# HuiHuiLan/Clustering-Hidden-Markov-Models-with-Variational-Bayesian-Hierarchical-EM

Measured on AMD Instinct MI355X. Metric: VBHEM E-steps/sec (whole node), N baseHMMs × K clusters × S states; ELBO match, higher is better.
Workload: dtype f64; 1 GPU; C4: N=100000 base HMMs, K=16 clusters, S=8 states, Sb=8, d=8, full cov, tau=10, Nv=100; N=100000, K=16, S=8, Sb=8, d=8, tau=10, parallelism=bases sharded over 1 GPU(s), 1 RCCL all-reduce/E-step

## Files before the change

### clustering-hidden-markov-models-with-variational-bayesian-hierarchical-em_amd/csrc/vbhem_em.hip

```cpp
#include <hip/hip_runtime.h>

#include <cfloat>
#include <chrono>
#include <cmath>
#include <cstdlib>
#include <map>
#include <mutex>
#include <string>
#include <vector>

#include "vbhem_em.h"
#include "vbhem_em_deriv_terms.h"
#include "vbhem_em_dev.h"
#include "vbhem_em_host.h"
#include "vbhem_em_trial_ctrl.h"
#include "vbhem_internal.h"
#include "vbhem_special.h"

namespace {

constexpr double kPi = 3.14159265358979323846;

using vbhem::psi_recur;

// ... 596 lines not shown
    if (std::isnan(L)) {
      L = -INFINITY;
      *stable = 0;
      break;
    }
    bool do_break = false;
    if (it > 1 && std::fabs((L - lastL) / lastL) <= opt->minDiff) do_break = true;
    if (it == opt->max_iter) do_break = true;
    LogLs[it] = L;
    ++it;
    lastL = L;
    if (do_break) break;
  }
  *iters = it;
  *L_final = L;
  if (deriv) {
    if (*stable) return derivs_at(&pre.t, opt, ext->dLL);
    nan_derivs(opt, d, ext->dLL);
  }
  return VBHEM_OK;
}

using MappedBuf = vbhem::EmMappedBuf;
std::map<int, std::vector<MappedBuf>> g_mapped_bufs;

hipError_t acquire_mapped_buf(size_t bytes, MappedBuf &m) {
  int dev = 0;
  hipError_t e = hipGetDevice(&dev);
  if (e != hipSuccess) return e;
  {
    std::lock_guard<std::mutex> g(g_mapped_mu);
    auto &v = g_mapped_bufs[dev];
    for (size_t x = 0; x < v.size(); ++x)
      if (v[x].bytes >= bytes) {
        m = v[x];
        v.erase(v.begin() + (long)x);
        return hipSuccess;
      }
    if (!v.empty()) {
      (void)hipHostFree(v.back().h);
      v.pop_back();
    }
  }
  m.bytes = (bytes + 4095) / 4096 * 4096;
  e = hipHostMalloc(reinterpret_cast<void **>(&m.h), m.bytes, hipHostMallocMapped);
  if (e == hipSuccess) e = hipHostGetDevicePointer(reinterpret_cast<void **>(&m.d), m.h, 0);
  return e;
}

void release_mapped_buf(const MappedBuf &m) {
  if (!m.h) return;
  int dev = 0;
  if (hipGetDevice(&dev) != hipSuccess) return;
  std::lock_guard<std::mutex> g(g_mapped_mu);
  g_mapped_bufs[dev].push_back(m);
}

size_t post_len(int K, int S, int d, size_t dd) {
  return (size_t)K + 3 * (size_t)K * S + (size_t)K * S * S + (size_t)K * S * d + (size_t)K * S * dd;
}

size_t trials_ws_doubles(int N, int K, int S, int d, size_t dd, int R, size_t slen, int nW) {
  const size_t KS = (size_t)K * S, nd = (size_t)VBHEM_DLL_LEN(d, nW);
  const size_t consts = KS * S + KS + KS * d + KS * dd + KS + (size_t)K;
  return (size_t)R * (2 * consts + 2 * post_len(K, S, d, dd) + 2 * KS + KS * 13 + 2 * slen +
                      2 * (size_t)N * K + (size_t)vbhem::hyp_table_len(d) + nd * KS + nd) +
         ((size_t)R * sizeof(vbhem::TrialCtrl) + 7) / 8 + ((size_t)R * sizeof(int) + 7) / 8;
}

const char *trials_unsupported(const vbhem_base_t *base, int K, int S, int R) {
  if (R < 1 || K < 1 || S < 1) return "R, KT and S must be positive";
  if ((long long)R * K > 256) return "R * KT > 256 (vbhem_estep_fused_trials)";
  if (S > 16) return "S > 16 (vbhem_estep_fused_trials)";
  if (base->SB > S) return "Sb > S (vbhem_estep_fused_trials)";
  if (!vbhem::em_dev_supported(base->d, S)) return "d > 16 (the device-side EM math)";
  return nullptr;
}

}

extern "C++" {
namespace vbhem {
hipError_t em_wait_flag(const int *flag, int seq, hipStream_t st) { return wait_flag(flag, seq, st); }
hipError_t em_acquire_mapped_buf(size_t bytes, EmMappedBuf &m) { return acquire_mapped_buf(bytes, m); }
void em_release_mapped_buf(const EmMappedBuf &m) { release_mapped_buf(m); }
}
}

int vbhem_em_run_ext(const vbhem_base_t *base, const double *tildeN_dev, int T,
                     const vbhem_em_opt_t *opt, vbhem_post_t *post, double *LogLs, int *iters,
                     double *L_final, int *stable, double *stats_dev, double *hatZ_dev,
                     double *LL_dev, void *workspace_dev, size_t workspace_bytes, void *stream,
                     vbhem_allreduce_fn allreduce, void *allreduce_ctx, const vbhem_em_ext_t *ext) {
  if (!base || !post_ok(post) || !opt_ok(opt, post->d) || !LogLs || !iters || !L_final ||
      !stable || !stats_dev || post->d != base->d || post->covmode != base->covmode)
    return VBHEM_ERR_ARG;
  if (ext && ext->rccl_comm && allreduce)
    return vbhem::set_error(VBHEM_ERR_ARG, "vbhem_em_run_ext: an RCCL communicator and an all-reduce callback");
  const int K = post->K, S = post->S, d = post->d;
  const size_t dd = post->covmode == VBHEM_COV_FULL ? (size_t)d * d : (size_t)d;
  const size_t need = vbhem_em_workspace_bytes(base, K, S, T);
  if (need == 0 || !workspace_dev || workspace_bytes < need) return VBHEM_ERR_WORKSPACE;
  hipStream_t st = static_cast<hipStream_t>(stream);
  if (!vbhem::em_dev_supported(d, S) || vbhem::switches().EM_HOST_MATH)
    return em_run_host(base, tildeN_dev, T, opt, post, LogLs, iters, L_final, stable, stats_dev,
                       hatZ_dev, LL_dev, workspace_dev, st, allreduce, allreduce_ctx, ext);
  vbhem_cluster_t c0 = {K, S, nullptr, nullptr, nullptr, nullptr, nullptr};
  const size_t fused = (vbhem_fused_workspace_bytes(base, &c0, T) + 255) / 256 * 256;
  const size_t nA = (size_t)K * S * S, nPi = (size_t)K * S, nm = (size_t)K * S * d,
               nP = (size_t)K * S * dd, nc = (size_t)K * S;
  double *dc = reinterpret_cast<double *>(static_cast<char *>(workspace_dev) + fused);
  vbhem_cluster_t cl = {K, S, dc, dc + nA, dc + nA + nPi, dc + nA + nPi + nm,
                        dc + nA + nPi + nm + nP};
  double *dlogOmega = dc + nA + nPi + nm + nP + nc;
  double *p = dlogOmega + K;
  PostDev pd[3];
  for (int x = 0; x < 3; ++x) pd[x] = carve_post(p, K, S, d, dd);
  double *dlLT = p; p += nc;
  double *dlogdetW = p; p += nc;
  double *dm0 = p; p += d;
  double *dW0inv = p; p += (size_t)d * d;
  double *dpart = p; p += (size_t)K * S * 13;
  int *dticket = reinterpret_cast<int *>(p); p += 1;
  double *hz[2] = {hatZ_dev, p}, *ll[2] = {LL_dev, p + (size_t)base->N * K};
  std::vector<double> W0inv;
  w0_inv(opt, d, W0inv);
  vbhem::EmDevArgs a{};
  a.K = K; a.S = S; a.d = d; a.covmode = post->covmode; a.NU = (int)vbhem_stats_nu(d, post->covmode);
  a.stats = stats_dev;
  a.alpha0 = opt->alpha0; a.eta0 = opt->eta0; a.epsilon0 = opt->epsilon0; a.lambda0 = opt->lambda0;
  a.v0 = opt->v0;
  bound_constants(opt, K, S, d, W0inv, a.logCalpha0, a.logCeta0, a.logCepsilon0, a.logB0);
  a.m0 = dm0; a.W0inv = dW0inv;
  a.logA = dc; a.logPi = dc + nA; a.cm = dc + nA + nPi; a.P = dc + nA + nPi + nm;
  a.c = dc + nA + nPi + nm + nP; a.lLT = dlLT; a.logOmega = dlogOmega; a.logdetW = dlogdetW;
  a.part = dpart; a.ticket = dticket;
  hipError_t e = hipMemcpyAsync(dm0, opt->m0, d * sizeof(double), hipMemcpyHostToDevice, st);
  if (e == hipSuccess)
    e = hipMemcpyAsync(dW0inv, W0inv.data(), W0inv.size() * sizeof(double), hipMemcpyHostToDevice, st);
  if (e == hipSuccess) e = copy_post(post, pd[0], dd, hipMemcpyHostToDevice, st);
  if (e == hipSuccess) e = hipMemsetAsync(dticket, 0, sizeof(int), st);
  Mapped mb;
  if (e == hipSuccess) e = acquire_mapped(mb);
  double *Lh = mb.h, *Ld = mb.d;
  int *flag_h = Lh ? reinterpret_cast<int *>(Lh + 2) : nullptr;
  if (flag_h) flag_h[0] = flag_h[1] = 0;
  auto set_post = [&a](const PostDev &in, const PostDev &out) {
    a.alpha = in.alpha; a.eta = in.eta; a.eps = in.eps; a.lam = in.lam; a.v = in.v; a.m = in.m;
    a.W = in.W;
    a.alpha_o = out.alpha; a.eta_o = out.eta; a.eps_o = out.eps; a.lam_o = out.lam; a.v_o = out.v;
    a.m_o = out.m; a.W_o = out.W;
  };
  set_post(pd[0], pd[1]);
  if (e == hipSuccess) e = vbhem::launch_em_dev(a, vbhem::kEmPrelude, nullptr, st);
  const size_t slen = vbhem_stats_len(K, S, d, post->covmode);
  int rc = VBHEM_OK;
  auto enqueue = [&](int j) -> bool {
    rc = vbhem_estep_fused(base, &cl, T, tildeN_dev, dlogOmega, stats_dev, hz[j % 2], ll[j % 2],
                           workspace_dev, fused, st);
    if (rc != VBHEM_OK) return false;
    rc = reduce_stats(ext, allreduce, allreduce_ctx, stats_dev, slen, st);
    if (rc != VBHEM_OK) return false;
    set_post(pd[j % 3], pd[(j + 1) % 3]);
    a.seq = j + 1;
    a.flag = reinterpret_cast<int *>(Ld + 2) + (j % 2);
    void *t0 = vbhem::timing_begin(st);
    e = vbhem::launch_em_dev(a, vbhem::kEmIterate, Ld + (j % 2), st);
    vbhem::timing_end_em_math(t0, st);
    return e == hipSuccess;
  };
  double lastL = -DBL_MAX, L = -INFINITY;
  int it = 0, fin_post = 0, fin_e = 0;
  *stable = 1;
  bool ok = e == hipSuccess && enqueue(0);
  while (ok) {
    if (it + 1 <= opt->max_iter && !enqueue(it + 1)) break;
    e = wait_flag(flag_h + (it % 2), it + 1, st);
    if (e != hipSuccess) break;
    if (ext && ext->iter_seconds) ext->iter_seconds[it] = now_s();
    L = Lh[it % 2];
    fin_e = it % 2;
    if (std::isnan(L)) {
      L = -INFINITY;
      *stable = 0;
      fin_post = it % 3;
      break;
    }
    bool do_break = false;
    if (it > 1 && std::fabs((L - lastL) / lastL) <= opt->minDiff) do_break = true;
    if (it == opt->max_iter) do_break = true;
    LogLs[it] = L;
    ++it;
    lastL = L;
    fin_post = it % 3;
    if (do_break) break;
  }
  hipError_t e2 = hipStreamSynchronize(st);
  if (e == hipSuccess) e = e2;
  if (e == hipSuccess && rc == VBHEM_OK && fin_e == 1 && base->N > 0) {
    e = hipMemcpyAsync(hatZ_dev, hz[1], (size_t)base->N * K * sizeof(double),
                       hipMemcpyDeviceToDevice, st);
    if (e == hipSuccess)
      e = hipMemcpyAsync(LL_dev, ll[1], (size_t)base->N * K * sizeof(double),
                         hipMemcpyDeviceToDevice, st);
  }
  const bool deriv = ext && ext->calc_deriv && ext->dLL;
  HostPost pre;
  if (deriv && *stable && it >= 1) pre.size_like(post);
  if (e == hipSuccess && rc == VBHEM_OK) e = copy_post(post, pd[fin_post], dd, hipMemcpyDeviceToHost, st);
  if (e == hipSuccess && rc == VBHEM_OK && deriv && *stable && it >= 1)
    e = copy_post(&pre.t, pd[(it - 1) % 3], dd, hipMemcpyDeviceToHost, st);
  if (e == hipSuccess && rc == VBHEM_OK) e = hipStreamSynchronize(st);
  if (e == hipSuccess) release_mapped(mb);
  if (rc != VBHEM_OK) return rc;
  if (e != hipSuccess) return VBHEM_ERR_HIP;
  *iters = it;
  *L_final = L;
  if (deriv) {
    if (*stable && it >= 1) return derivs_at(&pre.t, opt, ext->dLL);
    nan_derivs(opt, d, ext->dLL);
  }
  return VBHEM_OK;
}

int vbhem_em_run(const vbhem_base_t *base, const double *tildeN_dev, int T,
                 const vbhem_em_opt_t *opt, vbhem_post_t *post, double *LogLs, int *iters,
                 double *L_final, int *stable, double *stats_dev, double *hatZ_dev,
                 double *LL_dev, void *workspace_dev, size_t workspace_bytes, void *stream,
                 vbhem_allreduce_fn allreduce, void *allreduce_ctx) {
  return vbhem_em_run_ext(base, tildeN_dev, T, opt, post, LogLs, iters, L_final, stable, stats_dev,
                          hatZ_dev, LL_dev, workspace_dev, workspace_bytes, stream, allreduce,
                          allreduce_ctx, nullptr);
}

size_t vbhem_em_trials_hyp_workspace_bytes(const vbhem_base_t *base, int KT, int S, int R, int T,
                                           int W0_len) {
  if (!base || trials_unsupported(base, KT, S, R)) return 0;
  const int d = base->d;
  if (W0_len != 1 && W0_len != d) return 0;
  const size_t dd = base->covmode == VBHEM_COV_FULL ? (size_t)d * d : (size_t)d;
  vbhem_cluster_t c = {R * KT, S, nullptr, nullptr, nullptr, nullptr, nullptr};
  const size_t fused = vbhem_fused_trials_workspace_bytes(base, &c, R, T);
  if (fused == 0) return 0;
  const size_t slen = vbhem_stats_len(KT, S, d, base->covmode);
  return (fused + 255) / 256 * 256 +
         trials_ws_doubles(base->N, KT, S, d, dd, R, slen, W0_len) * sizeof(double) + 256;
}

size_t vbhem_em_trials_workspace_bytes(const vbhem_base_t *base, int KT, int S, int R, int T) {
  return base ? vbhem_em_trials_hyp_workspace_bytes(base, KT, S, R, T, base->d) : 0;
}

static int run_trials_impl(const char *fn, const vbhem_base_t *base, const double *tildeN_dev, int R,
                           int T, const vbhem_em_opt_t *const *opts, const int *active,
                           vbhem_post_t *posts, double *LogLs, int *iters, double *L_final,
                           int *stable, double *stats_out, double *hatZ_dev, double *LL_dev,
                           double *dLL, void *workspace_dev, size_t workspace_bytes, void *stream) {
  const std::string who = std::string(fn) + ": ";
  if (!base || !posts || R < 1 || !post_ok(&posts[0]) || !opts || !opt_ok(opts[0], posts[0].d) ||
      !LogLs || !iters || !L_final || !stable || !stats_out || !hatZ_dev || !LL_dev || !tildeN_dev)
    return vbhem::set_error(VBHEM_ERR_ARG, who + "null or invalid argument");
  const vbhem_em_opt_t *opt = opts[0];
  const int K = posts[0].K, S = posts[0].S, d = posts[0].d, cov = posts[0].covmode;
  if (d != base->d || cov != base->covmode)
    return vbhem::set_error(VBHEM_ERR_ARG, who + "d / covmode differ from the base set's");
  for (int r = 1; r < R; ++r) {
    if (!opt_ok(opts[r], d)) return vbhem::set_error(VBHEM_ERR_ARG, who + "null or invalid argument");
    if (opts[r]->max_iter != opt->max_iter || opts[r]->minDiff != opt->minDiff ||
        opts[r]->Nv != opt->Nv || opts[r]->W0_len != opt->W0_len)
      return vbhem::set_error(VBHEM_ERR_ARG,
                              who + "max_iter, minDiff, Nv and W0_len must be equal in every trial's options");
  }
  if (const char *why = trials_unsupported(base, K, S, R))
    return vbhem::set_error(VBHEM_ERR_UNSUPPORTED, who + why);
  for (int r = 1; r < R; ++r)
    if (!post_ok(&posts[r]) || posts[r].K != K || posts[r].S != S || posts[r].d != d ||
        posts[r].covmode != cov)
      return vbhem::set_error(VBHEM_ERR_ARG, who + "the trials' posteriors differ in shape");
  const int nW = opt->W0_len, nd = VBHEM_DLL_LEN(d, nW);
  const size_t need = vbhem_em_trials_hyp_workspace_bytes(base, K, S, R, T, nW);
  if (need == 0)
    return vbhem::set_error(VBHEM_ERR_UNSUPPORTED, who + "no batched E-step for this shape");
  if (!workspace_dev || workspace_bytes < need) return VBHEM_ERR_WORKSPACE;
  hipStream_t st = static_cast<hipStream_t>(stream);
  const int N = base->N, RK = R * K;
  const size_t dd = cov == VBHEM_COV_FULL ? (size_t)d * d : (size_t)d, KS = (size_t)K * S;
  vbhem_cluster_t c0 = {RK, S, nullptr, nullptr, nullptr, nullptr, nullptr};
  const size_t fused = (vbhem_fused_trials_workspace_bytes(base, &c0, R, T) + 255) / 256 * 256;
  const size_t slen = vbhem_stats_len(K, S, d, cov), postn = post_len(K, S, d, dd);
  const size_t nA = KS * S, nPi = KS, nm = KS * d, nP = KS * dd, nc = KS, nO = (size_t)K;
  const size_t consts = (size_t)R * (nA + nPi + nm + nP + nc + nO);
  double *p = reinterpret_cast<double *>(static_cast<char *>(workspace_dev) + fused);
  double *dc = p; p += consts;
  double *dbackup = p; p += consts;
  double *dposts = p; p += 2 * (size_t)R * postn;
  double *dlLT = p; p += (size_t)R * KS;
  double *dlogdetW = p; p += (size_t)R * KS;
  double *dpart = p; p += (size_t)R * KS * 13;
  double *dstats = p; p += (size_t)R * slen;
  double *dstats_out = p; p += (size_t)R * slen;
  double *dhz = p; p += (size_t)N * RK;
  double *dll = p; p += (size_t)N * RK;
  const size_t hlen = (size_t)vbhem::hyp_table_len(d);
  double *dhyp = p; p += (size_t)R * hlen;
  double *dterms = p; p += (size_t)R * nd * KS;
  double *ddLL = p; p += (size_t)R * nd;
  vbhem::TrialCtrl *dctrl = reinterpret_cast<vbhem::TrialCtrl *>(p);
  p += ((size_t)R * sizeof(vbhem::TrialCtrl) + 7) / 8;
  int *dticket = reinterpret_cast<int *>(p);
  vbhem_cluster_t cl = {RK, S, dc, dc + R * nA, dc + R * (nA + nPi), dc + R * (nA + nPi + nm),
                        dc + R * (nA + nPi + nm + nP)};
  double *dlogOmega = dc + R * (nA + nPi + nm + nP + nc);

  std::vector<double> hyp((size_t)R * hlen), W0inv;
  for (int r = 0; r < R; ++r) {
    const vbhem_em_opt_t *o = opts[r];
    double *h = hyp.data() + (size_t)r * hlen;
    if (r > 0 && o == opts[r - 1]) {
      std::copy(h - hlen, h, h);
      continue;
// ... 169 lines not shown
```

### clustering-hidden-markov-models-with-variational-bayesian-hierarchical-em_amd/csrc/vbhem_em_dev.h

```cpp
#pragma once
#include <hip/hip_runtime.h>

namespace vbhem {

constexpr int kEmDevMaxD = 16;

enum { kEmPrelude = 0, kEmIterate = 1 };

struct EmDevArgs {
  int K, S, d, covmode, NU;
  const double *alpha, *eta, *eps, *lam, *v, *m, *W;
  double *alpha_o, *eta_o, *eps_o, *lam_o, *v_o, *m_o, *W_o;
  const double *stats;
  double alpha0, eta0, epsilon0, lambda0, v0;
  double logCalpha0, logCeta0, logCepsilon0, logB0;
  const double *m0;
  const double *W0inv;
  double *logA, *logPi, *cm, *P, *c, *lLT, *logOmega, *logdetW;
  double *part;
  int *ticket;
  int *flag;
  int seq;
};

bool em_dev_supported(int d, int S);
hipError_t launch_em_dev(const EmDevArgs &a, int mode, double *L_out, hipStream_t st);

struct TrialCtrl;

struct EmTrialsArgs {
  EmDevArgs a;
  int R, N;
  size_t postn;
  size_t stats_len;
  TrialCtrl *ctrl;
  int *ticket;
  double *LogLs;
  int ldL, max_iter;
  double minDiff;
  double *backup;
  const double *hz, *ll;
  double *hz_out, *ll_out;
  double *stats_out;
  int *flag, *active;
  const double *hyp;
  size_t hyp_stride;
  int W0_len;
  double *dterms, *dLL;
};

hipError_t launch_em_trials(const EmTrialsArgs &t, int mode, hipStream_t st);
hipError_t launch_trials_latch(const EmTrialsArgs &t, int j, hipStream_t st);
hipError_t launch_trials_derivs(const EmTrialsArgs &t, hipStream_t st);

}
```

### clustering-hidden-markov-models-with-variational-bayesian-hierarchical-em_amd/csrc/vbhem_em_dev.hip

```cpp
#include <hip/hip_runtime.h>

#include <cmath>

#include "vbhem_em_dev.h"
#include "vbhem_special.h"

#ifdef EMDEV_TIMING
namespace vbhem {
namespace {
__device__ long long emdev_t[8][1024];
}
}
#define EMDEV_MARK(ph)                                                  \
  if (lane == 0 && ks < 1024) emdev_t[ph][ks] = __builtin_amdgcn_s_memrealtime()
#endif
#include "vbhem_em_iter_body.h"

namespace vbhem {

namespace {

__global__ __launch_bounds__(64 * kWaves) void em_iter_kernel(const EmDevArgs a, int mode,
                                                              double *L_out) {
  __shared__ double glds[kWaves][2 * kEmDevMaxD * kEmDevMaxD];
  const int lane = threadIdx.x & 63, wave = threadIdx.x >> 6;
  const int K = a.K, S = a.S;
  const int ks = __builtin_amdgcn_readfirstlane(blockIdx.x * kWaves + wave);
  if (ks >= K * S) return;
  const bool iterate = mode == kEmIterate;
  const StatsView st(a.stats, K, S);
  EMDEV_MARK(0);
  em_ks_body(a, iterate, ks, lane, glds[wave], st);

  EMDEV_MARK(6);
  if (iterate) {
    __builtin_amdgcn_fence(__ATOMIC_RELEASE, "agent");
    int last = 0;
    if (lane == 0) last = atomicAdd(a.ticket, 1) == K * S - 1;
    last = __shfl(last, 0, 64);
    if (last) {
      __builtin_amdgcn_fence(__ATOMIC_ACQUIRE, "agent");
      const double L = em_bound_total(a, st, lane);
      if (lane == 0) {
        *L_out = L;
        *a.ticket = 0;
        EMDEV_MARK(7);
        if (a.flag) {
          __threadfence_system();
          __hip_atomic_store(a.flag, a.seq, __ATOMIC_RELEASE, __HIP_MEMORY_SCOPE_SYSTEM);
        }
      }
    }
  }
}

}

bool em_dev_supported(int d, int S) { return d >= 1 && d <= kEmDevMaxD && S >= 1 && S <= 32; }

hipError_t launch_em_dev(const EmDevArgs &a, int mode, double *L_out, hipStream_t st) {
  if (!em_dev_supported(a.d, a.S) || (mode == kEmIterate && (!L_out || !a.ticket || !a.part)))
    return hipErrorInvalidValue;
  const int nw = a.K * a.S;
  hipLaunchKernelGGL(em_iter_kernel, dim3((nw + kWaves - 1) / kWaves), dim3(64 * kWaves), 0, st, a,
                     mode, L_out);
  return hipGetLastError();
}

}
```

### clustering-hidden-markov-models-with-variational-bayesian-hierarchical-em_amd/csrc/vbhem_em_iter_body.h

```cpp
#pragma once
#include <hip/hip_runtime.h>

#include <cmath>

#include "vbhem_em_dev.h"
#include "vbhem_special.h"

#ifndef EMDEV_MARK
#define EMDEV_MARK(ph)
#endif

namespace vbhem {

namespace {

constexpr double kPiD = 3.14159265358979323846;
constexpr double kLn2D = 0.69314718055994530942;
constexpr int kWaves = 4;

__device__ __forceinline__ void wsync() {
  __builtin_amdgcn_fence(__ATOMIC_RELEASE, "wavefront");
  __builtin_amdgcn_wave_barrier();
  __builtin_amdgcn_fence(__ATOMIC_ACQUIRE, "wavefront");
}

template <int CTRL, int ROWS>
__device__ __forceinline__ double dpp_d(double v) {
  const int lo = __builtin_amdgcn_update_dpp(0, __double2loint(v), CTRL, ROWS, 0xf, true);
  const int hi = __builtin_amdgcn_update_dpp(0, __double2hiint(v), CTRL, ROWS, 0xf, true);
  return __hiloint2double(hi, lo);
}

__device__ __forceinline__ double wsum(double v) {
  v += dpp_d<0x111, 0xf>(v);
  v += dpp_d<0x112, 0xf>(v);
  v += dpp_d<0x114, 0xf>(v);
  v += dpp_d<0x118, 0xf>(v);
  v += dpp_d<0x142, 0xa>(v);
  v += dpp_d<0x143, 0xc>(v);
  const int lo = __builtin_amdgcn_readlane(__double2loint(v), 63);
  const int hi = __builtin_amdgcn_readlane(__double2hiint(v), 63);
  return __hiloint2double(hi, lo);
}

__device__ __forceinline__ double gauss_jordan(double *g, int d, int cols, int lane) {
  const int w2 = 2 * d, n = d * cols;
  int er[8], ec[8];
#pragma unroll
  for (int j = 0; j < 8; ++j) {
    const int x = lane + 64 * j;
    er[j] = x < n ? x / cols : -1;
    ec[j] = x < n ? x - er[j] * cols : 0;
  }
  double det = 1.0;
  for (int k = 0; k < d; ++k) {
    const double piv = g[k * w2 + k], rp = 1.0 / piv;
    double nv[8];
#pragma unroll
    for (int j = 0; j < 8; ++j) {
      if (er[j] >= 0) {
        const int r = er[j], c = ec[j];
        const double rk = g[k * w2 + c] * rp;
        nv[j] = r == k ? rk : fma(-g[r * w2 + k], rk, g[r * w2 + c]);
      }
    }
    det *= piv;
    wsync();
#pragma unroll
    for (int j = 0; j < 8; ++j)
      if (er[j] >= 0) g[er[j] * w2 + ec[j]] = nv[j];
    wsync();
  }
  return det;
}

struct StatsView {
  const double *Nj, *N1, *M, *U;
  double Lt1, Lt7;
  __device__ StatsView(const double *v, int K, int S) {
    Nj = N1 = M = U = nullptr;
    Lt1 = Lt7 = 0.0;
    if (!v) return;
    size_t o = 0;
    Nj = v + o; o += K;
    N1 = v + o; o += (size_t)K * S;
    M = v + o; o += (size_t)K * S * S;
    Lt1 = v[o];
    Lt7 = v[o + 1];
    o += 2;
    U = v + o;
  }
};

constexpr int kNQ = 13;

__device__ __forceinline__ void em_ks_body(const EmDevArgs &a, const bool iterate, const int ks,
                                           const int lane, double *g, const StatsView &st) {
  const int K = a.K, S = a.S, d = a.d;
  const int k = ks / S, s = ks - k * S;
  const bool full = a.covmode == 1;
  const int dd = full ? d * d : d;
  if (iterate) {
    const double v = a.v[ks], lam = a.lam[ks], lLT = a.lLT[ks], l0 = a.lambda0;
    const double *W = a.W + (size_t)ks * dd, *mk = a.m + (size_t)ks * d;
    double t_eps = 0.0, t_ept = 0.0, t_la = 0.0;
    if (lane >= 32 && lane - 32 < S) {
      const int s2 = lane - 32;
      const double la = a.logA[(size_t)ks * S + s2];
      t_eps = a.eps[(size_t)ks * S + s2];
      t_ept = (t_eps - 1) * la;
      t_la = la;
    }
    const double e = a.eta[ks];
    double es = 0.0, lo = 0.0, al = 0.0;
    if (s == 0) {
      es = wsum(lane < S ? a.eta[(size_t)k * S + lane] : 0.0);
      lo = a.logOmega[k];
      al = a.alpha[k];
    }
    const double ps = wsum(t_eps);
    double xg = 0.0;
    bool lg_on = false;
    if (lane < d) {
      xg = 0.5 * (v - lane);
      lg_on = true;
    } else if (lane >= 32 && lane - 32 < S) {
      xg = t_eps;
      lg_on = true;
    } else if (lane >= 16 && lane < 20) {
      xg = lane == 16 ? ps : lane == 17 ? e : lane == 18 ? es : al;
      lg_on = lane < 18 || s == 0;
    }
    const double lgx = lg_on ? lgamma_stirling(xg) : 0.0;
    double t_mwm = 0.0, t_tr = 0.0;
    for (int x = lane; x < d * d; x += 64) {
      const int r = x / d, c = x - r * d;
      const double wrc = full ? W[x] : (r == c ? W[r] : 0.0);
      const double wcr = full ? W[c * d + r] : wrc;
      t_mwm += (mk[r] - a.m0[r]) * wrc * (mk[c] - a.m0[c]);
      t_tr += a.W0inv[x] * wcr;
    }
    const double sg = wsum(lane < d ? lgx : 0.0), lgp = wsum(lane >= 32 ? lgx : 0.0);
    const double pt = wsum(t_ept), sla = wsum(t_la), mWm = wsum(t_mwm), trW = wsum(t_tr);
    const double lg_ps = __shfl(lgx, 16, 64), lg_e = __shfl(lgx, 17, 64);
    const double lg_es = __shfl(lgx, 18, 64), lg_al = __shfl(lgx, 19, 64);
    if (lane < kNQ) {
      const double logBk = -(v / 2) * a.logdetW[ks] - (v * d / 2) * kLn2D -
                           (d * (d - 1) / 4.0) * log(kPiD) - sg;
      double q = 0.0;
      switch (lane) {
        case 0: q = d * log(l0 / (2 * kPiD)) + lLT - d * l0 / lam - l0 * v * mWm; break;
        case 1: q = lLT; break;
        case 2: q = v * trW; break;
        case 3: q = lLT + d * log(lam / (2 * kPiD)); break;
        case 4: q = -logBk - 0.5 * (v - d - 1) * lLT + 0.5 * v * d; break;
        case 5: q = lg_ps - lgp + pt - lg_e + (e - 1) * a.logPi[ks] + (s == 0 ? lg_es : 0.0); break;
        case 6: q = a.logPi[ks]; break;
        case 7: q = sla; break;
        case 8: q = s == 0 ? (st.Nj[k] + 1e-50) * lo : 0.0; break;
        case 9: q = s == 0 ? lo : 0.0; break;
        case 10: q = s == 0 ? (al - 1) * lo : 0.0; break;
        case 11: q = s == 0 ? lg_al : 0.0; break;
        default: q = s == 0 ? al : 0.0; break;
      }
      a.part[(size_t)lane * K * S + ks] = q;
    }
  }

  EMDEV_MARK(1);
  const int w2 = 2 * d;
  double v, lam, m_l = 0.0, e_l = 0.0, eta_ks, sum_eta = 0.0, alpha_k, det_mt = 1.0;
  if (iterate) {
    const double *u = st.U + (size_t)ks * a.NU;
    const double Nr = u[0] + 1e-50, l0 = a.lambda0;
    lam = l0 + Nr;
    v = a.v0 + Nr + 1.0;
    const double mult1 = l0 * Nr / (l0 + Nr);
    for (int x = lane; x < d * w2; x += 64) {
      const int r = x / w2, c = x - r * w2;
      double val;
      if (c < d) {
        const double yr = u[1 + r] / Nr, yc = u[1 + c] / Nr;
        double sc;
        if (full) {
          const int lo = r < c ? r : c, hi = r < c ? c : r;
          sc = u[1 + d + lo * d - lo * (lo - 1) / 2 + (hi - lo)] / Nr - yr * yc;
        } else {
          sc = r == c ? u[1 + d + r] / Nr - yr * yr : 0.0;
        }
        val = a.W0inv[r * d + c] + Nr * sc + mult1 * (yr - a.m0[r]) * (yc - a.m0[c]);
      } else {
        val = (c - d == r) ? 1.0 : 0.0;
      }
      g[x] = val;
    }
    if (lane < d) {
      m_l = (l0 * a.m0[lane] + Nr * (u[1 + lane] / Nr)) / (l0 + Nr);
      a.m_o[(size_t)ks * d + lane] = m_l;
    }
    if (lane == 0) {
      a.lam_o[ks] = lam;
      a.v_o[ks] = v;
    }
    wsync();
    EMDEV_MARK(2);
    det_mt = gauss_jordan(g, d, 2 * d, lane);
    EMDEV_MARK(3);
    double nw[4];
#pragma unroll
    for (int j = 0; j < 4; ++j) {
      const int x = lane + 64 * j;
      if (x < d * d) {
        const int r = x / d, c = x - r * d;
        nw[j] = (g[r * w2 + d + c] + g[c * w2 + d + r]) / 2;
      }
    }
    wsync();
    double *Wo = a.W_o + (size_t)ks * dd;
#pragma unroll
    for (int j = 0; j < 4; ++j) {
      const int x = lane + 64 * j;
      if (x < d * d) {
        const int r = x / d, c = x - r * d;
        g[r * w2 + c] = full ? nw[j] : (r == c ? nw[j] : 0.0);
        g[r * w2 + d + c] = r == c ? 1.0 : 0.0;
        if (full) Wo[x] = nw[j];
        else if (r == c) Wo[r] = nw[j];
      }
    }
    eta_ks = a.eta0 + st.N1[ks];
    if (lane < S) sum_eta = a.eta0 + st.N1[(size_t)k * S + lane];
    const int s2 = lane & 31;
    if (s2 < S) {
      e_l = a.epsilon0 + (S > 1 ? st.M[(size_t)ks * S + s2] : 1e-12);
      if (lane < 32) a.eps_o[(size_t)ks * S + s2] = e_l;
    }
    if (lane == 0) a.eta_o[ks] = eta_ks;
    alpha_k = a.alpha0 + (st.Nj[k] + 1e-50);
    if (s == 0 && lane == 0) a.alpha_o[k] = alpha_k;
  } else {
    v = a.v[ks];
    lam = a.lam[ks];
    eta_ks = a.eta[ks];
    if (lane < S) sum_eta = a.eta[(size_t)k * S + lane];
    if (lane < d) m_l = a.m[(size_t)ks * d + lane];
    if ((lane & 31) < S) e_l = a.eps[(size_t)ks * S + (lane & 31)];
    alpha_k = a.alpha[k];
    const double *W = a.W + (size_t)ks * dd;
    for (int x = lane; x < d * w2; x += 64) {
      const int r = x / w2, c = x - r * w2;
      g[x] = c < d ? (full ? W[r * d + c] : (r == c ? W[r] : 0.0)) : ((c - d == r) ? 1.0 : 0.0);
    }
  }
  wsync();
  EMDEV_MARK(4);
  sum_eta = wsum(lane < S ? sum_eta : 0.0);

  const double es = wsum(lane >= 32 && lane - 32 < S ? e_l : 0.0);
  double sa = 0.0;
  if (s == 0) {
    double t = 0.0;
    for (int j = lane; j < K; j += 64)
      t += iterate ? a.alpha0 + (st.Nj[j] + 1e-50) : a.alpha[j];
    sa = wsum(t);
  }
  double xp = 0.0;
  bool p_on = false;
  if (lane < d) {
    xp = 0.5 * (v - lane);
    p_on = true;
  } else if (lane >= 32 && lane - 32 < S) {
    xp = e_l;
    p_on = true;
  } else if (lane >= 16 && lane < 21) {
    xp = lane == 16 ? es : lane == 17 ? eta_ks : lane == 18 ? sum_eta : lane == 19 ? alpha_k : sa;
    p_on = lane < 19 || s == 0;
  }
  const double pl = p_on ? psi_onediv(xp) : 0.0;
  const double t1 = wsum(lane < d ? pl : 0.0);
  const double pes = __shfl(pl, 16, 64), pet = __shfl(pl, 17, 64), pst = __shfl(pl, 18, 64);
  const double pal = __shfl(pl, 19, 64), psa = __shfl(pl, 20, 64);
  for (int x = lane; x < dd; x += 64) {
    const int r = full ? x / d : x, c = full ? x - r * d : x;
    a.P[(size_t)ks * dd + x] = v * g[r * w2 + c];
  }
  double logdet;
  if (full && iterate) {
    logdet = -log(det_mt);
  } else if (full) {
    wsync();
    logdet = log(gauss_jordan(g, d, d, lane));
  } else {
    logdet = wsum(lane < d ? log(g[lane * w2 + lane]) : 0.0);
  }
  EMDEV_MARK(5);
  const double lLT = t1 + d * kLn2D + logdet;
  if (lane < d) a.cm[(size_t)ks * d + lane] = m_l;
  if (lane >= 32 && lane - 32 < S) a.logA[(size_t)ks * S + (lane - 32)] = pl - pes;
  if (lane == 0) {
    a.lLT[ks] = lLT;
    a.logdetW[ks] = logdet;
    a.c[ks] = -lLT + d / lam;
    a.logPi[ks] = pet - pst;
    if (s == 0) a.logOmega[k] = pal - psa;
  }
}

__device__ __forceinline__ double em_bound_total(const EmDevArgs &a, const StatsView &st,
                                                 const int lane) {
  const int K = a.K, S = a.S, d = a.d;
  double q[kNQ];
#pragma unroll
  for (int x = 0; x < kNQ; ++x) q[x] = 0.0;
  for (int j = lane; j < K * S; j += 64) {
#pragma unroll
    for (int x = 0; x < kNQ; ++x) q[x] += a.part[(size_t)x * K * S + j];
  }
#pragma unroll
  for (int x = 0; x < kNQ; ++x) q[x] = wsum(q[x]);
  double L = 0.0;
  if (lane == 0) {
    const double a0 = a.alpha0, e0 = a.eta0, ep0 = a.epsilon0, v0 = a.v0;
    const double Lt3 = K * a.logCeta0 + (e0 - 1) * q[6];
    const double Lt4 = (double)K * S * a.logCepsilon0 + (ep0 - 1) * q[7];
    const double Lt5 =
        0.5 * q[0] + (double)K * S * a.logB0 + 0.5 * (v0 - d - 1) * q[1] - 0.5 * q[2];
    const double Lt6 = a.logCalpha0 + (a0 - 1) * q[9];
    const double Lt8 = (lgamma_stirling(q[12]) - q[11]) + q[10];
    const double Lt10 = 0.5 * q[3] - 0.5 * d * S * K - q[4];
    L = st.Lt1 + q[8] + Lt3 + Lt4 + Lt5 + Lt6 - st.Lt7 - Lt8 - q[5] - Lt10;
  }
  return L;
}

}

}
```

### clustering-hidden-markov-models-with-variational-bayesian-hierarchical-em_amd/csrc/vbhem_switches.h

```cpp
#pragma once

#define VBHEM_SWITCHES(X)                                                                      \
  X(FUSED_DENSE, 0, "dense schedule instead of the gated one (vbhem_set_fused_mode)")          \
  X(NO_UGEMM, 0, "emission on the raw / generic kernels instead of the prepared operand")      \
  X(GROUP_BASES, -1, "tests: at most n bases per group of the fused call")                     \
  X(NSLAB, -1, "tests: at most n statistics slabs (1 .. 8192)")                                \
  X(NO_BWD2, 0, "backward pass on fb_split_kernel's backward mode, not fb_bwd2_kernel")        \
  X(NO_BWD4, 0, "S = 8: fb_bwd2_kernel<8> instead of fb_bwd4_kernel")                          \
  X(NO_BWD12, 0, "S = 12: fb_bwd2_kernel<12> instead of fb_bwd12_kernel")                      \
  X(NO_LIST4, 0, "S = 8: fb_split_kernel's list mode instead of fb_list4_kernel")              \
  X(NO_LIST12, 0, "S = 12: fb_split_kernel's list mode instead of fb_list12_kernel")           \
  X(NO_K1_IN_KERNEL, 0, "short K1 through the emission GEMM, not inside the recursion")        \
  X(NO_LIST4_STATS, 0, "S = 8: per-pair outputs + stats_list_m_kernel, not sums in fb_list4_kernel") \
  X(NO_LIST_INLINE, 0, "the gate-list pass's flagged pairs through an fb_exact_kernel launch") \
  X(NO_BWD2_PREP, 0, "emission_prep_kernel launched, not its work inside fb_bwd2_kernel")      \
  X(NO_FOLD_EXACT, 0, "the backward pass's fallback as a launch, not folded into resp_kernel") \
  X(EM_NOBST, 0, "the one-chunk emission GEMM without buffer stores")                          \
  X(EM_SPLIT, -1, "the one-chunk emission GEMM in whole (0) or half (1) tiles")                \
  X(EM_NODB, 0, "the chunked emission GEMM on emission_u_kernel, not emission_db_kernel")      \
  X(RESP_GENERIC, 0, "resp_kernel's generic path for every K")                                 \
  X(NO_GATE_MASKS, 0, "K <= 64: gate_list_kernel re-reads Z, not the responsibility kernel's gate masks") \
  X(NO_FINAL_FOLD, 0, "list4_stats_reduce_kernel launched, not folded into the finishing kernel") \
  X(SU_BLOCKS, -1, "gated statistics: the block count")                                        \
  X(NO_STATS_G, 0, "gated statistics: no lane-grouped kernel")                                 \
  X(NO_STATS_U, 0, "gated statistics: the covariance-gather kernel")                           \
  X(NO_STATS_M, 0, "gated statistics: without stats_list_m_kernel")                            \
  X(EM_HOST_MATH, 0, "the EM loop's per-iteration math on the host")

namespace vbhem {

struct Switches {
#define X(name, unset, doc) long long name = unset;
  VBHEM_SWITCHES(X)
#undef X
};

const Switches &switches();

}
```

Baseline: 584.4 E-steps/s.

## Split per-(k,s) EM update across specialized waves in one block

Adds em_iter_mw_kernel, which gives each cluster-state pair its own block of waves instead of one wave. One wave runs the Gauss-Jordan posterior chain, another computes the bound partial terms and takes the completion ticket, and a third does the digamma terms, all in parallel, with shared-memory handoff for the tail. The last block's final bound reduction is also spread across waves. The aim is to shorten the serial latency of the small EM M-step kernel (K*S=128 pairs) inside the E-step loop, at the cost of more blocks and a block barrier. The old kernel stays reachable through the EM_ONE_WAVE switch.

```diff
diff --git a/clustering-hidden-markov-models-with-variational-bayesian-hierarchical-em_amd/csrc/vbhem_em.hip b/clustering-hidden-markov-models-with-variational-bayesian-hierarchical-em_amd/csrc/vbhem_em.hip
--- a/clustering-hidden-markov-models-with-variational-bayesian-hierarchical-em_amd/csrc/vbhem_em.hip
+++ b/clustering-hidden-markov-models-with-variational-bayesian-hierarchical-em_amd/csrc/vbhem_em.hip
@@ -772,7 +772,8 @@
     a.m_o = out.m; a.W_o = out.W;
   };
   set_post(pd[0], pd[1]);
-  if (e == hipSuccess) e = vbhem::launch_em_dev(a, vbhem::kEmPrelude, nullptr, st);
+  const bool one_wave = vbhem::switches().EM_ONE_WAVE != 0;
+  if (e == hipSuccess) e = vbhem::launch_em_dev(a, vbhem::kEmPrelude, nullptr, st, one_wave);
   const size_t slen = vbhem_stats_len(K, S, d, post->covmode);
   int rc = VBHEM_OK;
   auto enqueue = [&](int j) -> bool {
@@ -785,7 +786,7 @@
     a.seq = j + 1;
     a.flag = reinterpret_cast<int *>(Ld + 2) + (j % 2);
     void *t0 = vbhem::timing_begin(st);
-    e = vbhem::launch_em_dev(a, vbhem::kEmIterate, Ld + (j % 2), st);
+    e = vbhem::launch_em_dev(a, vbhem::kEmIterate, Ld + (j % 2), st, one_wave);
     vbhem::timing_end_em_math(t0, st);
     return e == hipSuccess;
   };
diff --git a/clustering-hidden-markov-models-with-variational-bayesian-hierarchical-em_amd/csrc/vbhem_em_dev.h b/clustering-hidden-markov-models-with-variational-bayesian-hierarchical-em_amd/csrc/vbhem_em_dev.h
--- a/clustering-hidden-markov-models-with-variational-bayesian-hierarchical-em_amd/csrc/vbhem_em_dev.h
+++ b/clustering-hidden-markov-models-with-variational-bayesian-hierarchical-em_amd/csrc/vbhem_em_dev.h
@@ -24,7 +24,8 @@
 };
 
 bool em_dev_supported(int d, int S);
-hipError_t launch_em_dev(const EmDevArgs &a, int mode, double *L_out, hipStream_t st);
+hipError_t launch_em_dev(const EmDevArgs &a, int mode, double *L_out, hipStream_t st,
+                         bool one_wave = false);
 
 struct TrialCtrl;
 
diff --git a/clustering-hidden-markov-models-with-variational-bayesian-hierarchical-em_amd/csrc/vbhem_em_dev.hip b/clustering-hidden-markov-models-with-variational-bayesian-hierarchical-em_amd/csrc/vbhem_em_dev.hip
--- a/clustering-hidden-markov-models-with-variational-bayesian-hierarchical-em_amd/csrc/vbhem_em_dev.hip
+++ b/clustering-hidden-markov-models-with-variational-bayesian-hierarchical-em_amd/csrc/vbhem_em_dev.hip
@@ -8,11 +8,15 @@
 #ifdef EMDEV_TIMING
 namespace vbhem {
 namespace {
-__device__ long long emdev_t[8][1024];
+__device__ long long emdev_t[9][1024];
 }
 }
 #define EMDEV_MARK(ph)                                                  \
   if (lane == 0 && ks < 1024) emdev_t[ph][ks] = __builtin_amdgcn_s_memrealtime()
+#define EMDEV_MARKW(w, ph)                                              \
+  if (threadIdx.x == 64 * (w) && ks < 1024) emdev_t[ph][ks] = __builtin_amdgcn_s_memrealtime()
+#else
+#define EMDEV_MARKW(w, ph)
 #endif
 #include "vbhem_em_iter_body.h"
 
@@ -54,16 +58,69 @@
   }
 }
 
+__global__ __launch_bounds__(64 * kMwWaves) void em_iter_mw_kernel(const EmDevArgs a, int mode,
+                                                                   double *L_out) {
+  __shared__ MwShared sh;
+  const int lane = threadIdx.x & 63;
+  const int wave = __builtin_amdgcn_readfirstlane(threadIdx.x >> 6);
+  const int K = a.K, S = a.S;
+  const int ks = blockIdx.x;
+  const bool iterate = mode == kEmIterate;
+  const StatsView st(a.stats, K, S);
+  double logdet = 0.0, lam = 1.0, m_l = 0.0, pl = 0.0;
+  EMDEV_MARKW(kMwChain, 0);
+  if (wave == kMwChain) {
+    em_mw_chain(a, iterate, ks, lane, sh.g, st, logdet, lam, m_l);
+    EMDEV_MARKW(kMwChain, 5);
+  } else if (wave == kMwBound) {
+    int last = 0;
+    if (iterate) {
+      em_bound_terms(a, ks, lane, st);
+      asm volatile("s_waitcnt vmcnt(0)" ::: "memory");
+      __builtin_amdgcn_fence(__ATOMIC_RELEASE, "agent");
+      asm volatile("s_waitcnt vmcnt(0)" ::: "memory");
+      if (lane == 0) last = atomicAdd(a.ticket, 1) == K * S - 1;
+      if (last) __builtin_amdgcn_fence(__ATOMIC_ACQUIRE, "agent");
+    }
+    if (lane == 0) sh.last = last;
+    EMDEV_MARKW(kMwBound, 1);
+  } else if (wave == kMwPsi) {
+    pl = em_mw_psi(a, iterate, ks, lane, st, &sh.t1);
+    EMDEV_MARKW(kMwPsi, 8);
+  }
+  __syncthreads();
+  if (wave == kMwChain) em_mw_chain_tail(a, ks, lane, sh.t1, logdet, lam, m_l);
+  else if (wave == kMwPsi) em_mw_psi_tail(a, ks, lane, pl);
+  EMDEV_MARKW(kMwChain, 6);
+  if (!sh.last) return;
+  __builtin_amdgcn_fence(__ATOMIC_ACQUIRE, "agent");
+  em_mw_bound_sums(a, wave, lane, sh);
+  __syncthreads();
+  if (threadIdx.x == 0) {
+    *L_out = em_bound_formula(a, st, sh.q, sh.lg);
+    *a.ticket = 0;
+    EMDEV_MARKW(kMwChain, 7);
+    if (a.flag) {
+      __threadfence_system();
+      __hip_atomic_store(a.flag, a.seq, __ATOMIC_RELEASE, __HIP_MEMORY_SCOPE_SYSTEM);
+    }
+  }
+}
+
 }
 
 bool em_dev_supported(int d, int S) { return d >= 1 && d <= kEmDevMaxD && S >= 1 && S <= 32; }
 
-hipError_t launch_em_dev(const EmDevArgs &a, int mode, double *L_out, hipStream_t st) {
+hipError_t launch_em_dev(const EmDevArgs &a, int mode, double *L_out, hipStream_t st,
+                         bool one_wave) {
   if (!em_dev_supported(a.d, a.S) || (mode == kEmIterate && (!L_out || !a.ticket || !a.part)))
     return hipErrorInvalidValue;
   const int nw = a.K * a.S;
-  hipLaunchKernelGGL(em_iter_kernel, dim3((nw + kWaves - 1) / kWaves), dim3(64 * kWaves), 0, st, a,
-                     mode, L_out);
+  if (one_wave)
+    hipLaunchKernelGGL(em_iter_kernel, dim3((nw + kWaves - 1) / kWaves), dim3(64 * kWaves), 0, st,
+                       a, mode, L_out);
+  else
+    hipLaunchKernelGGL(em_iter_mw_kernel, dim3(nw), dim3(64 * kMwWaves), 0, st, a, mode, L_out);
   return hipGetLastError();
 }
 
diff --git a/clustering-hidden-markov-models-with-variational-bayesian-hierarchical-em_amd/csrc/vbhem_em_iter_body.h b/clustering-hidden-markov-models-with-variational-bayesian-hierarchical-em_amd/csrc/vbhem_em_iter_body.h
--- a/clustering-hidden-markov-models-with-variational-bayesian-hierarchical-em_amd/csrc/vbhem_em_iter_body.h
+++ b/clustering-hidden-markov-models-with-variational-bayesian-hierarchical-em_amd/csrc/vbhem_em_iter_body.h
@@ -94,78 +94,85 @@
 
 constexpr int kNQ = 13;
 
+__device__ __forceinline__ void em_bound_terms(const EmDevArgs &a, const int ks, const int lane,
+                                               const StatsView &st) {
+  const int K = a.K, S = a.S, d = a.d;
+  const int k = ks / S, s = ks - k * S;
+  const bool full = a.covmode == 1;
+  const int dd = full ? d * d : d;
+  const double v = a.v[ks], lam = a.lam[ks], lLT = a.lLT[ks], l0 = a.lambda0;
+  const double *W = a.W + (size_t)ks * dd, *mk = a.m + (size_t)ks * d;
+  double t_eps = 0.0, t_ept = 0.0, t_la = 0.0;
+  if (lane >= 32 && lane - 32 < S) {
+    const int s2 = lane - 32;
+    const double la = a.logA[(size_t)ks * S + s2];
+    t_eps = a.eps[(size_t)ks * S + s2];
+    t_ept = (t_eps - 1) * la;
+    t_la = la;
+  }
+  const double e = a.eta[ks];
+  double es = 0.0, lo = 0.0, al = 0.0;
+  if (s == 0) {
+    es = wsum(lane < S ? a.eta[(size_t)k * S + lane] : 0.0);
+    lo = a.logOmega[k];
+    al = a.alpha[k];
+  }
+  const double ps = wsum(t_eps);
+  double xg = 0.0;
+  bool lg_on = false;
+  if (lane < d) {
+    xg = 0.5 * (v - lane);
+    lg_on = true;
+  } else if (lane >= 32 && lane - 32 < S) {
+    xg = t_eps;
+    lg_on = true;
+  } else if (lane >= 16 && lane < 20) {
+    xg = lane == 16 ? ps : lane == 17 ? e : lane == 18 ? es : al;
+    lg_on = lane < 18 || s == 0;
+  }
+  const double lgx = lg_on ? lgamma_stirling(xg) : 0.0;
+  double t_mwm = 0.0, t_tr = 0.0;
+  for (int x = lane; x < d * d; x += 64) {
+    const int r = x / d, c = x - r * d;
+    const double wrc = full ? W[x] : (r == c ? W[r] : 0.0);
+    const double wcr = full ? W[c * d + r] : wrc;
+    t_mwm += (mk[r] - a.m0[r]) * wrc * (mk[c] - a.m0[c]);
+    t_tr += a.W0inv[x] * wcr;
+  }
+  const double sg = wsum(lane < d ? lgx : 0.0), lgp = wsum(lane >= 32 ? lgx : 0.0);
+  const double pt = wsum(t_ept), sla = wsum(t_la), mWm = wsum(t_mwm), trW = wsum(t_tr);
+  const double lg_ps = __shfl(lgx, 16, 64), lg_e = __shfl(lgx, 17, 64);
+  const double lg_es = __shfl(lgx, 18, 64), lg_al = __shfl(lgx, 19, 64);
+  if (lane < kNQ) {
+    const double logBk = -(v / 2) * a.logdetW[ks] - (v * d / 2) * kLn2D -
+                         (d * (d - 1) / 4.0) * log(kPiD) - sg;
+    double q = 0.0;
+    switch (lane) {
+      case 0: q = d * log(l0 / (2 * kPiD)) + lLT - d * l0 / lam - l0 * v * mWm; break;
+      case 1: q = lLT; break;
+      case 2: q = v * trW; break;
+      case 3: q = lLT + d * log(lam / (2 * kPiD)); break;
+      case 4: q = -logBk - 0.5 * (v - d - 1) * lLT + 0.5 * v * d; break;
+      case 5: q = lg_ps - lgp + pt - lg_e + (e - 1) * a.logPi[ks] + (s == 0 ? lg_es : 0.0); break;
+      case 6: q = a.logPi[ks]; break;
+      case 7: q = sla; break;
+      case 8: q = s == 0 ? (st.Nj[k] + 1e-50) * lo : 0.0; break;
+      case 9: q = s == 0 ? lo : 0.0; break;
+      case 10: q = s == 0 ? (al - 1) * lo : 0.0; break;
+      case 11: q = s == 0 ? lg_al : 0.0; break;
+      default: q = s == 0 ? al : 0.0; break;
+    }
+    a.part[(size_t)lane * K * S + ks] = q;
+  }
+}
+
 __device__ __forceinline__ void em_ks_body(const EmDevArgs &a, const bool iterate, const int ks,
                                            const int lane, double *g, const StatsView &st) {
   const int K = a.K, S = a.S, d = a.d;
   const int k = ks / S, s = ks - k * S;
   const bool full = a.covmode == 1;
   const int dd = full ? d * d : d;
-  if (iterate) {
-    const double v = a.v[ks], lam = a.lam[ks], lLT = a.lLT[ks], l0 = a.lambda0;
-    const double *W = a.W + (size_t)ks * dd, *mk = a.m + (size_t)ks * d;
-    double t_eps = 0.0, t_ept = 0.0, t_la = 0.0;
-    if (lane >= 32 && lane - 32 < S) {
-      const int s2 = lane - 32;
-      const double la = a.logA[(size_t)ks * S + s2];
-      t_eps = a.eps[(size_t)ks * S + s2];
-      t_ept = (t_eps - 1) * la;
-      t_la = la;
-    }
-    const double e = a.eta[ks];
-    double es = 0.0, lo = 0.0, al = 0.0;
-    if (s == 0) {
-      es = wsum(lane < S ? a.eta[(size_t)k * S + lane] : 0.0);
-      lo = a.logOmega[k];
-      al = a.alpha[k];
-    }
-    const double ps = wsum(t_eps);
-    double xg = 0.0;
-    bool lg_on = false;
-    if (lane < d) {
-      xg = 0.5 * (v - lane);
-      lg_on = true;
-    } else if (lane >= 32 && lane - 32 < S) {
-      xg = t_eps;
-      lg_on = true;
-    } else if (lane >= 16 && lane < 20) {
-      xg = lane == 16 ? ps : lane == 17 ? e : lane == 18 ? es : al;
-      lg_on = lane < 18 || s == 0;
-    }
-    const double lgx = lg_on ? lgamma_stirling(xg) : 0.0;
-    double t_mwm = 0.0, t_tr = 0.0;
-    for (int x = lane; x < d * d; x += 64) {
-      const int r = x / d, c = x - r * d;
-      const double wrc = full ? W[x] : (r == c ? W[r] : 0.0);
-      const double wcr = full ? W[c * d + r] : wrc;
-      t_mwm += (mk[r] - a.m0[r]) * wrc * (mk[c] - a.m0[c]);
-      t_tr += a.W0inv[x] * wcr;
-    }
-    const double sg = wsum(lane < d ? lgx : 0.0), lgp = wsum(lane >= 32 ? lgx : 0.0);
-    const double pt = wsum(t_ept), sla = wsum(t_la), mWm = wsum(t_mwm), trW = wsum(t_tr);
-    const double lg_ps = __shfl(lgx, 16, 64), lg_e = __shfl(lgx, 17, 64);
-    const double lg_es = __shfl(lgx, 18, 64), lg_al = __shfl(lgx, 19, 64);
-    if (lane < kNQ) {
-      const double logBk = -(v / 2) * a.logdetW[ks] - (v * d / 2) * kLn2D -
-                           (d * (d - 1) / 4.0) * log(kPiD) - sg;
-      double q = 0.0;
-      switch (lane) {
-        case 0: q = d * log(l0 / (2 * kPiD)) + lLT - d * l0 / lam - l0 * v * mWm; break;
-        case 1: q = lLT; break;
-        case 2: q = v * trW; break;
-        case 3: q = lLT + d * log(lam / (2 * kPiD)); break;
-        case 4: q = -logBk - 0.5 * (v - d - 1) * lLT + 0.5 * v * d; break;
-        case 5: q = lg_ps - lgp + pt - lg_e + (e - 1) * a.logPi[ks] + (s == 0 ? lg_es : 0.0); break;
-        case 6: q = a.logPi[ks]; break;
-        case 7: q = sla; break;
-        case 8: q = s == 0 ? (st.Nj[k] + 1e-50) * lo : 0.0; break;
-        case 9: q = s == 0 ? lo : 0.0; break;
-        case 10: q = s == 0 ? (al - 1) * lo : 0.0; break;
-        case 11: q = s == 0 ? lg_al : 0.0; break;
-        default: q = s == 0 ? al : 0.0; break;
-      }
-      a.part[(size_t)lane * K * S + ks] = q;
-    }
-  }
+  if (iterate) em_bound_terms(a, ks, lane, st);
 
   EMDEV_MARK(1);
   const int w2 = 2 * d;
@@ -306,9 +313,23 @@
   }
 }
 
+__device__ __forceinline__ double em_bound_formula(const EmDevArgs &a, const StatsView &st,
+                                                   const double *q, const double lg_sum_alpha) {
+  const int K = a.K, S = a.S, d = a.d;
+  const double a0 = a.alpha0, e0 = a.eta0, ep0 = a.epsilon0, v0 = a.v0;
+  const double Lt3 = K * a.logCeta0 + (e0 - 1) * q[6];
+  const double Lt4 = (double)K * S * a.logCepsilon0 + (ep0 - 1) * q[7];
+  const double Lt5 =
+      0.5 * q[0] + (double)K * S * a.logB0 + 0.5 * (v0 - d - 1) * q[1] - 0.5 * q[2];
+  const double Lt6 = a.logCalpha0 + (a0 - 1) * q[9];
+  const double Lt8 = (lg_sum_alpha - q[11]) + q[10];
+  const double Lt10 = 0.5 * q[3] - 0.5 * d * S * K - q[4];
+  return st.Lt1 + q[8] + Lt3 + Lt4 + Lt5 + Lt6 - st.Lt7 - Lt8 - q[5] - Lt10;
+}
+
 __device__ __forceinline__ double em_bound_total(const EmDevArgs &a, const StatsView &st,
                                                  const int lane) {
-  const int K = a.K, S = a.S, d = a.d;
+  const int K = a.K, S = a.S;
   double q[kNQ];
 #pragma unroll
   for (int x = 0; x < kNQ; ++x) q[x] = 0.0;
@@ -319,20 +340,216 @@
 #pragma unroll
   for (int x = 0; x < kNQ; ++x) q[x] = wsum(q[x]);
   double L = 0.0;
+  if (lane == 0) L = em_bound_formula(a, st, q, lgamma_stirling(q[12]));
+  return L;
+}
+
+constexpr int kMwWaves = 4;
+enum { kMwChain = 0, kMwBound = 1, kMwPsi = 2 };
+
+struct MwShared {
+  double g[2 * kEmDevMaxD * kEmDevMaxD];
+  double t1;
+  double q[kNQ], lg;
+  int last;
+};
+
+__device__ __forceinline__ void em_mw_chain(const EmDevArgs &a, const bool iterate, const int ks,
+                                            const int lane, double *g, const StatsView &st,
+                                            double &logdet, double &lam, double &m_l) {
+  const int d = a.d, w2 = 2 * d;
+  const bool full = a.covmode == 1;
+  const int dd = full ? d * d : d;
+  double v, det_mt = 1.0;
+  m_l = 0.0;
+  if (iterate) {
+    const double *u = st.U + (size_t)ks * a.NU;
+    const double Nr = u[0] + 1e-50, l0 = a.lambda0;
+    lam = l0 + Nr;
+    v = a.v0 + Nr + 1.0;
+    const double mult1 = l0 * Nr / (l0 + Nr);
+    for (int x = lane; x < d * w2; x += 64) {
+      const int r = x / w2, c = x - r * w2;
+      double val;
+      if (c < d) {
+        const double yr = u[1 + r] / Nr, yc = u[1 + c] / Nr;
+        double sc;
+        if (full) {
+          const int lo = r < c ? r : c, hi = r < c ? c : r;
+          sc = u[1 + d + lo * d - lo * (lo - 1) / 2 + (hi - lo)] / Nr - yr * yc;
+        } else {
+          sc = r == c ? u[1 + d + r] / Nr - yr * yr : 0.0;
+        }
+        val = a.W0inv[r * d + c] + Nr * sc + mult1 * (yr - a.m0[r]) * (yc - a.m0[c]);
+      } else {
+        val = (c - d == r) ? 1.0 : 0.0;
+      }
+      g[x] = val;
+    }
+    if (lane < d) {
+      m_l = (l0 * a.m0[lane] + Nr * (u[1 + lane] / Nr)) / (l0 + Nr);
+      a.m_o[(size_t)ks * d + lane] = m_l;
+    }
+    if (lane == 0) {
+      a.lam_o[ks] = lam;
+      a.v_o[ks] = v;
+    }
+    wsync();
+    EMDEV_MARK(2);
+    det_mt = gauss_jordan(g, d, 2 * d, lane);
+    EMDEV_MARK(3);
+    double nw[4];
+#pragma unroll
+    for (int j = 0; j < 4; ++j) {
+      const int x = lane + 64 * j;
+      if (x < d * d) {
+        const int r = x / d, c = x - r * d;
+        nw[j] = (g[r * w2 + d + c] + g[c * w2 + d + r]) / 2;
+      }
+    }
+    wsync();
+    double *Wo = a.W_o + (size_t)ks * dd;
+#pragma unroll
+    for (int j = 0; j < 4; ++j) {
+      const int x = lane + 64 * j;
+      if (x < d * d) {
+        const int r = x / d, c = x - r * d;
+        g[r * w2 + c] = full ? nw[j] : (r == c ? nw[j] : 0.0);
+        if (full) Wo[x] = nw[j];
+        else if (r == c) Wo[r] = nw[j];
+      }
+    }
+  } else {
+    v = a.v[ks];
+    lam = a.lam[ks];
+    if (lane < d) m_l = a.m[(size_t)ks * d + lane];
+    const double *W = a.W + (size_t)ks * dd;
+    for (int x = lane; x < d * w2; x += 64) {
+      const int r = x / w2, c = x - r * w2;
+      g[x] = c < d ? (full ? W[r * d + c] : (r == c ? W[r] : 0.0)) : ((c - d == r) ? 1.0 : 0.0);
+    }
+  }
+  wsync();
+  EMDEV_MARK(4);
+  for (int x = lane; x < dd; x += 64) {
+    const int r = full ? x / d : x, c = full ? x - r * d : x;
+    a.P[(size_t)ks * dd + x] = v * g[r * w2 + c];
+  }
+  if (full && iterate) {
+    logdet = -log(det_mt);
+  } else if (full) {
+    wsync();
+    logdet = log(gauss_jordan(g, d, d, lane));
+  } else {
+    logdet = wsum(lane < d ? log(g[lane * w2 + lane]) : 0.0);
+  }
+}
+
+__device__ __forceinline__ void em_mw_chain_tail(const EmDevArgs &a, const int ks, const int lane,
+                                                 const double t1, const double logdet,
+                                                 const double lam, const double m_l) {
+  const int d = a.d;
+  const double lLT = t1 + d * kLn2D + logdet;
+  if (lane < d) a.cm[(size_t)ks * d + lane] = m_l;
   if (lane == 0) {
-    const double a0 = a.alpha0, e0 = a.eta0, ep0 = a.epsilon0, v0 = a.v0;
-    const double Lt3 = K * a.logCeta0 + (e0 - 1) * q[6];
-    const double Lt4 = (double)K * S * a.logCepsilon0 + (ep0 - 1) * q[7];
-    const double Lt5 =
-        0.5 * q[0] + (double)K * S * a.logB0 + 0.5 * (v0 - d - 1) * q[1] - 0.5 * q[2];
-    const double Lt6 = a.logCalpha0 + (a0 - 1) * q[9];
-    const double Lt8 = (lgamma_stirling(q[12]) - q[11]) + q[10];
-    const double Lt10 = 0.5 * q[3] - 0.5 * d * S * K - q[4];
-    L = st.Lt1 + q[8] + Lt3 + Lt4 + Lt5 + Lt6 - st.Lt7 - Lt8 - q[5] - Lt10;
-  }
-  return L;
-}
-
-}
-
-}
+    a.lLT[ks] = lLT;
+    a.logdetW[ks] = logdet;
+    a.c[ks] = -lLT + d / lam;
+  }
+}
+
+__device__ __forceinline__ double em_mw_psi(const EmDevArgs &a, const bool iterate, const int ks,
+                                            const int lane, const StatsView &st, double *t1_out) {
+  const int K = a.K, S = a.S, d = a.d;
+  const int k = ks / S, s = ks - k * S;
+  double v, e_l = 0.0, eta_ks, sum_eta = 0.0, alpha_k;
+  if (iterate) {
+    const double Nr = st.U[(size_t)ks * a.NU] + 1e-50;
+    v = a.v0 + Nr + 1.0;
+    eta_ks = a.eta0 + st.N1[ks];
+    if (lane < S) sum_eta = a.eta0 + st.N1[(size_t)k * S + lane];
+    const int s2 = lane & 31;
+    if (s2 < S) {
+      e_l = a.epsilon0 + (S > 1 ? st.M[(size_t)ks * S + s2] : 1e-12);
+      if (lane < 32) a.eps_o[(size_t)ks * S + s2] = e_l;
+    }
+    if (lane == 0) a.eta_o[ks] = eta_ks;
+    alpha_k = a.alpha0 + (st.Nj[k] + 1e-50);
+    if (s == 0 && lane == 0) a.alpha_o[k] = alpha_k;
+  } else {
+    v = a.v[ks];
+    eta_ks = a.eta[ks];
+    if (lane < S) sum_eta = a.eta[(size_t)k * S + lane];
+    if ((lane & 31) < S) e_l = a.eps[(size_t)ks * S + (lane & 31)];
+    alpha_k = a.alpha[k];
+  }
+  sum_eta = wsum(lane < S ? sum_eta : 0.0);
+  const double es = wsum(lane >= 32 && lane - 32 < S ? e_l : 0.0);
+  double sa = 0.0;
+  if (s == 0) {
+    double t = 0.0;
+    for (int j = lane; j < K; j += 64)
+      t += iterate ? a.alpha0 + (st.Nj[j] + 1e-50) : a.alpha[j];
+    sa = wsum(t);
+  }
+  double xp = 0.0;
+  bool p_on = false;
+  if (lane < d) {
+    xp = 0.5 * (v - lane);
+    p_on = true;
+  } else if (lane >= 32 && lane - 32 < S) {
+    xp = e_l;
+    p_on = true;
+  } else if (lane >= 16 && lane < 21) {
+    xp = lane == 16 ? es : lane == 17 ? eta_ks : lane == 18 ? sum_eta : lane == 19 ? alpha_k : sa;
+    p_on = lane < 19 || s == 0;
+  }
+  const double pl = p_on ? psi_onediv(xp) : 0.0;
+  const double t1 = wsum(lane < d ? pl : 0.0);
+  if (lane == 0) *t1_out = t1;
+  return pl;
+}
+
+__device__ __forceinline__ void em_mw_psi_tail(const EmDevArgs &a, const int ks, const int lane,
+                                               const double pl) {
+  const int S = a.S;
+  const int k = ks / S, s = ks - k * S;
+  const double pes = __shfl(pl, 16, 64), pet = __shfl(pl, 17, 64), pst = __shfl(pl, 18, 64);
+  const double pal = __shfl(pl, 19, 64), psa = __shfl(pl, 20, 64);
+  if (lane >= 32 && lane - 32 < S) a.logA[(size_t)ks * S + (lane - 32)] = pl - pes;
+  if (lane == 0) {
+    a.logPi[ks] = pet - pst;
+    if (s == 0) a.logOmega[k] = pal - psa;
+  }
+}
+
+__device__ __forceinline__ void em_mw_bound_sums(const EmDevArgs &a, const int wave, const int lane,
+                                                 MwShared &sh) {
+  const int KS = a.K * a.S;
+  constexpr int kPer = (kNQ + kMwWaves - 1) / kMwWaves;
+  double t[kPer];
+#pragma unroll
+  for (int y = 0; y < kPer; ++y) t[y] = 0.0;
+  for (int j = lane; j < KS; j += 64) {
+#pragma unroll
+    for (int y = 0; y < kPer; ++y) {
+      const int x = wave + y * kMwWaves;
+      if (x < kNQ) t[y] += a.part[(size_t)x * KS + j];
+    }
+  }
+#pragma unroll
+  for (int y = 0; y < kPer; ++y) {
+    const int x = wave + y * kMwWaves;
+    if (x < kNQ) {
+      const double q = wsum(t[y]);
+      if (lane == 0) {
+        sh.q[x] = q;
+        if (x == kNQ - 1) sh.lg = lgamma_stirling(q);
+      }
+    }
+  }
+}
+
+}
+
+}
diff --git a/clustering-hidden-markov-models-with-variational-bayesian-hierarchical-em_amd/csrc/vbhem_switches.h b/clustering-hidden-markov-models-with-variational-bayesian-hierarchical-em_amd/csrc/vbhem_switches.h
--- a/clustering-hidden-markov-models-with-variational-bayesian-hierarchical-em_amd/csrc/vbhem_switches.h
+++ b/clustering-hidden-markov-models-with-variational-bayesian-hierarchical-em_amd/csrc/vbhem_switches.h
@@ -25,7 +25,8 @@
   X(NO_STATS_G, 0, "gated statistics: no lane-grouped kernel")                                 \
   X(NO_STATS_U, 0, "gated statistics: the covariance-gather kernel")                           \
   X(NO_STATS_M, 0, "gated statistics: without stats_list_m_kernel")                            \
-  X(EM_HOST_MATH, 0, "the EM loop's per-iteration math on the host")
+  X(EM_HOST_MATH, 0, "the EM loop's per-iteration math on the host")                          \
+  X(EM_ONE_WAVE, 0, "em_iter_kernel (one wave per cluster state), not em_iter_mw_kernel's block of waves")
 
 namespace vbhem {
 
```

Measured after the change: 584.4 E-steps/s (median of 2 runs). Within noise of the previous version (+0.0%).
